# maciejkula/spotlight

Hardware: AMD Instinct MI355X
Metric: training interactions/sec, BPR dim=64 (higher is better)
Workload: dtype f32

## Files before the change

### spotlight_amd/csrc/slk_api.hip

```cpp
#include <stdarg.h>

#include <stdlib.h>

#include "slk_common.h"

static char g_create_err[512] = {0};

int slk_fail(slk_ctx *ctx, int code, const char *fmt, ...) {
    char *dst = ctx ? ctx->err : g_create_err;
    va_list ap;
    va_start(ap, fmt);
    vsnprintf(dst, 512, fmt, ap);
    va_end(ap);
    return code;
}

int slk_ensure(slk_ctx *ctx, slk_buf &b, size_t bytes) {
    if (bytes <= b.cap) return SLK_OK;
    if (b.p) {
        SLK_HIP(ctx, hipFree(b.p));
        b.p = nullptr;
        b.cap = 0;
    }
    size_t want = bytes + bytes / 8 + 256;
// ... 185 lines not shown
    SLK_OPT("sort_big_min", opt_sort_big_min, 1, SLK_OPT_MAX),
    SLK_OPT("sort_debug", opt_sort_debug, 0, 3),
    SLK_OPT("item_grid_mult", opt_item_grid_mult, 1, 4096),
    SLK_OPT("user_grid_mult", opt_user_grid_mult, 1, 4096),
    SLK_OPT("seq_variant", opt_seq_variant, 0, 1),
    SLK_OPT("explicit_fused", opt_explicit_fused, 0, 1),
    SLK_OPT("epoch_kernel", opt_epoch_kernel, 0, 1),
    SLK_OPT("item_lat_max_tiles", opt_item_lat_max_tiles, 0, SLK_OPT_MAX),
    SLK_OPT("epoch_adaptive", opt_epoch_adaptive, 0, 1),
    SLK_OPT("epoch_adaptive_max_batch", opt_epoch_adaptive_max_batch, 1, (int64_t)1 << 20),
    SLK_OPT("epoch_max_batch", opt_epoch_max_batch, 1, (int64_t)1 << 20),
    SLK_OPT("epoch_max_grid", opt_epoch_max_grid, 1, 16384),
    SLK_OPT("epoch_barrier", opt_epoch_barrier, -1, 1),
    SLK_OPT("epoch_cooperative", opt_epoch_cooperative, 0, 1),
    SLK_OPT("epoch_debug", opt_epoch_debug, 0, 63),
    SLK_OPT("epoch_dense_elems", opt_epoch_dense_elems, 0, SLK_OPT_MAX),
    SLK_OPT("user_lat_max_batch", opt_user_lat_max_batch, 0, SLK_OPT_MAX),
    SLK_OPT("item_long_gate", opt_item_long_gate, 0, 1),
    SLK_OPT("adaptive_late_min_batch", opt_adaptive_late_min_batch, 0, SLK_OPT_MAX),
    SLK_OPT("shuffle_band", opt_shuffle_band, 0, 1024),
    SLK_OPT("nt", opt_nt, 0, 63),
    SLK_OPT("record_nt_min_bytes", opt_record_nt_min_bytes, 0, SLK_OPT_MAX),
    SLK_OPT("user_bias_zero_hint", opt_user_bias_zero_hint, 0, 1),
    SLK_OPT("user_grid_own_occ", opt_user_grid_own_occ, 0, 1),
    SLK_OPT("item_single_min_items", opt_item_single_min_items, 0, SLK_OPT_MAX),
};
#undef SLK_OPT
const slk_opt_desc slk_eval_options[] = {
    {"topk_items_per_wg", 0, (int64_t)1 << 40, [](const slk_ctx *c) -> int64_t { return c->opt_topk_items_per_wg; },
     [](slk_ctx *c, int64_t v) { c->opt_topk_items_per_wg = v; }},
    {"eval_items_per_wg", 0, (int64_t)1 << 40, [](const slk_ctx *c) -> int64_t { return c->opt_eval_items_per_wg; },
     [](slk_ctx *c, int64_t v) { c->opt_eval_items_per_wg = v; }},
};
const slk_opt_desc *slk_find_option(const char *name) {
    for (const slk_opt_desc &d : slk_options)
        if (!strcmp(name, d.name)) return &d;
    for (const slk_opt_desc &d : slk_eval_options)
        if (!strcmp(name, d.name)) return &d;
    return nullptr;
}
}

SLK_EXPORT int slk_ctx_set_option(slk_ctx *ctx, const char *name, int64_t value) {
    if (!ctx || !name) return SLK_EINVAL;
    const slk_opt_desc *d = slk_find_option(name);
    if (!d || value < d->lo || value > d->hi)
        return slk_fail(ctx, SLK_EINVAL, "slk_ctx_set_option: unknown option or bad value: %s = %lld", name,
                        (long long)value);
    d->set(ctx, value);
    return SLK_OK;
}

SLK_EXPORT int slk_ctx_get_option(slk_ctx *ctx, const char *name, int64_t *value) {
    if (!ctx || !name || !value) return SLK_EINVAL;
    const slk_opt_desc *d = slk_find_option(name);
    if (!d) return slk_fail(ctx, SLK_EINVAL, "slk_ctx_get_option: unknown option %s", name);
    *value = d->get(ctx);
    return SLK_OK;
}

SLK_EXPORT int slk_ctx_get_stat(slk_ctx *ctx, const char *name, int64_t *value) {
    if (!ctx || !name || !value) return SLK_EINVAL;
    if (!strcmp(name, "shuffle_sweeps")) *value = ctx->fy_sweeps;
    else if (!strcmp(name, "shuffle_fallbacks")) *value = ctx->fy_fallbacks;
    else if (!strcmp(name, "epoch_refused")) *value = ctx->epoch_refused ? 1 : 0;
    else if (!strcmp(name, "user_long_launches")) *value = ctx->stat_user_long;
    else if (!strcmp(name, "item_long_launches")) *value = ctx->stat_item_long;
    else if (!strcmp(name, "overlapped_chunks")) *value = ctx->stat_overlapped;
    else if (!strcmp(name, "prefetched_chunks")) *value = ctx->stat_prefetched;
    else if (!strcmp(name, "shadowed_calls")) *value = ctx->stat_shadowed;
    else if (!strcmp(name, "pingpong_calls")) *value = ctx->stat_pingpong;
    else if (!strcmp(name, "single_minibatches")) *value = ctx->stat_single;
    else if (!strcmp(name, "lds_per_block")) *value = (int64_t)ctx->lds_per_block;
    else if (!strcmp(name, "lds_per_cu")) *value = (int64_t)ctx->lds_per_cu;
    else if (!strcmp(name, "prefetch_pending")) *value = !ctx->pf.valid ? 0 : (ctx->pf.all ? 2 : 1);
    else return slk_fail(ctx, SLK_EINVAL, "slk_ctx_get_stat: unknown statistic %s", name);
    return SLK_OK;
}

SLK_EXPORT int slk_profile_enable(slk_ctx *ctx, int32_t on) {
    if (!ctx) return SLK_EINVAL;
    if (!on) slk_prof_drain(ctx);
    ctx->prof_on = on != 0;
    return SLK_OK;
}

SLK_EXPORT int slk_profile_read(slk_ctx *ctx, int32_t cls, int64_t *launches, double *total_ms) {
    if (!ctx || cls < 0 || cls >= SLK_K_COUNT) return SLK_EINVAL;
    int rc = slk_prof_drain(ctx);
    if (rc) return rc;
    if (launches) *launches = ctx->prof_launches[cls];
    if (total_ms) *total_ms = ctx->prof_ms[cls];
    return SLK_OK;
}

SLK_EXPORT int slk_profile_reset(slk_ctx *ctx) {
    if (!ctx) return SLK_EINVAL;
    int rc = slk_prof_drain(ctx);
    for (int i = 0; i < SLK_K_COUNT; ++i) {
        ctx->prof_launches[i] = 0;
        ctx->prof_ms[i] = 0.0;
    }
    return rc;
}
// ... 1 lines not shown
```

### spotlight_amd/csrc/slk_bilinear.hip

```cpp
#include <math.h>

#include "slk_kernels.h"

#ifndef SLK_PP_PIPE
#define SLK_PP_PIPE 2
#endif
template <int VEC, int G, int UPD, int UMODE, bool BLOOM, bool LAT = false, bool ULONG = false, bool PP = false, bool SGL = false>
__global__ __launch_bounds__(256) void k_user_pass(slk_pass_args a) {
    static_assert(!LAT || (UMODE == 0 && !BLOOM), "LAT is the pair mode over plain tables");
    static_assert(!PP || (UMODE == 0 && !BLOOM), "PP is the pair mode over plain tables");
    static_assert(!SGL || (PP && !LAT && !ULONG && UPD == SLK_UPD_ADAGRAD), "SGL: the plain ping-pong form, Adagrad");
    static_assert(!ULONG || !BLOOM, "long user runs: plain tables");
    constexpr uint32_t S = SLK_USER_TILE;
    constexpr bool PRE = UMODE != 0;
    constexpr bool EXPL = UMODE == 2;
    __shared__ double red[256];
    constexpr int GPB = 256 / G;
    const int lane = threadIdx.x % G;
    const int grp = threadIdx.x / G;
    const int D = a.D;
    const int d0 = lane * VEC;
    const bool on = d0 < D;
    const uint32_t stride = gridDim.x * GPB;
    float loss_acc = 0.0f;
// ... 1149 lines not shown

        if (nn == 0) return SLK_OK;
        if (d_neg_in) {
            slk_prof_begin(ctx, SLK_K_SAMPLE, s);
            hipLaunchKernelGGL(k_i64_to_u32, dim3(slk_grid_for(ctx, (size_t)nc * nn, 256)), dim3(256), 0, s,
                               d_neg_in + c0 * nn, neg32, (size_t)nc * nn);
            SLK_LAUNCH_CHECK(ctx, "k_i64_to_u32");
            if (d_neg_out)
                SLK_HIP(ctx, hipMemcpyAsync(d_neg_out + c0 * nn, d_neg_in + c0 * nn, (size_t)nc * nn * 8,
                                            hipMemcpyDeviceToDevice, s));
            slk_prof_end(ctx, s);
        } else {
            if ((rc = slk_sample_u32(ctx, tables->num_items, (int64_t)nc * nn, neg32,
                                     d_neg_out ? d_neg_out + c0 * nn : nullptr, s)))
                return rc;
        }
        return SLK_OK;
    };
    auto do_sort = [&](size_t ck, slk_prep_bufs &pb, hipStream_t s) -> int {
        int rc;
        const int64_t c0 = cb[ck];
        const uint32_t nc = (uint32_t)(cb[ck + 1] - c0);
        const uint32_t nocc = nc * (uint32_t)NP;
        const int64_t *cu = d_users + c0, *ci = d_items + c0;
        const uint32_t *neg32 = neg_all ? neg_all + (size_t)c0 * nn : (const uint32_t *)pb.neg32.p;

        slk_prof_begin(ctx, SLK_K_PREP, s);
        const unsigned mbbits = slk_bits_for((uint64_t)((nc - 1) / (uint32_t)bsz));
        uint32_t *ukey_in = (uint32_t *)pb.ukey[0].p, *ukey = (uint32_t *)pb.ukey[1].p;
        const uint32_t *uit, *uk = nullptr;
        uint32_t *const ukeys[2] = {ukey_in, ukey};
        if (!pre) {
            uint64_t *const uvals[2] = {(uint64_t *)pb.uval[0].p, (uint64_t *)pb.uval[1].p};
            if ((rc = slk_sort_user_fat(ctx, cu, ci, (const uint32_t *)neg32, nc, (size_t)bsz, ubits, mbbits, ukeys, uvals, s))) return rc;
            uit = (const uint32_t *)pb.uval[1].p;
        } else {
            uint32_t *const uvals[2] = {(uint32_t *)pb.uval[0].p, (uint32_t *)pb.uval[1].p};
            if ((rc = slk_sort_user_idx(ctx, cu, nc, (size_t)bsz, ubits, mbbits, ukeys, uvals, s))) return rc;
            uk = (const uint32_t *)pb.uval[1].p;
            hipLaunchKernelGGL(k_pack_items, dim3(slk_grid_for(ctx, nc, 256)), dim3(256), 0, s, uk, ci,
                               (const uint32_t *)neg32, nc, nn, (uint32_t *)pb.uit.p);
            SLK_LAUNCH_CHECK(ctx, "k_pack_items");
            uit = (const uint32_t *)pb.uit.p;
        }
        if (late) {
            hipLaunchKernelGGL(k_invert_perm, dim3(slk_grid_for(ctx, nc, 256)), dim3(256), 0, s, uk, nc,
                               (uint32_t *)pb.ipay[0].p);
            SLK_LAUNCH_CHECK(ctx, "k_invert_perm");
        } else {
            uint32_t *const ikeys[2] = {(uint32_t *)pb.ikey[0].p, (uint32_t *)pb.ikey[1].p};
            uint32_t *const ivals[2] = {(uint32_t *)pb.ipay[0].p, (uint32_t *)pb.ipay[1].p};
            if ((rc = slk_sort_item_occ(ctx, uit, nocc, (size_t)bsz, NP, ibits, mbbits, ikeys, ivals, s))) return rc;
            if (sgl_on) {
                SLK_HIP(ctx, hipMemsetAsync(pb.mflag.p, 0, (size_t)nocc, s));
                hipLaunchKernelGGL(k_item_multi_flags, dim3(slk_grid_for(ctx, nocc, 256)), dim3(256), 0, s, (const uint32_t *)pb.ikey[1].p,
                                   (const uint32_t *)pb.ipay[1].p, nocc, (uint32_t)bsz * (uint32_t)NP, (uint8_t *)pb.msorted.p,
                                   (uint8_t *)pb.mflag.p);
                SLK_LAUNCH_CHECK(ctx, "k_item_multi_flags");
            }
        }
        if (!epoch_route) {
            const uint32_t n_mb_c = (nc + (uint32_t)bsz - 1) / (uint32_t)bsz;
            if ((rc = slk_ensure(ctx, pb.lflags, 2 * (size_t)n_mb_c * 4))) return rc;
            SLK_HIP(ctx, hipMemsetAsync(pb.lflags.p, 0, 2 * (size_t)n_mb_c * 4, s));
            if (!late) {
                hipLaunchKernelGGL(k_item_long_flags, dim3(slk_grid_for(ctx, nocc / (4 * gpb) + n_mb_c, 256)), dim3(256), 0, s,
                                   (const uint32_t *)pb.ikey[1].p, nocc, (uint32_t)bsz * (uint32_t)NP, 4u * gpb,
// ... 494 lines not shown
```

### spotlight_amd/csrc/slk_common.h

```cpp
#pragma once
#include <hip/hip_runtime.h>
#include <stdint.h>
#include <stdio.h>
#include <string.h>

#include <vector>

#include "../../include/spotlight_hip.h"

#define SLK_EAGAIN_EPOCH 1
#define SLK_EXPORT extern "C" __attribute__((visibility("default")))

#if defined(__HIPCC__)
#define SLK_WAVES_PER_EU(n) __attribute__((amdgpu_waves_per_eu(n, n)))
#define SLK_WAVES_PER_EU_RANGE(lo, hi) __attribute__((amdgpu_waves_per_eu(lo, hi)))
#else
#define SLK_WAVES_PER_EU(n)
#define SLK_WAVES_PER_EU_RANGE(lo, hi)
#endif

#if defined(__HIPCC__)
#define SLK_DRAIN_VMEM() asm volatile("s_waitcnt vmcnt(0)" ::: "memory")
#else
#define SLK_DRAIN_VMEM() ((void)0)
// ... 55 lines not shown
    hipEvent_t a, b;
};

struct slk_ctx {
    int device = 0;
    int num_cus = 256;
    size_t lds_per_block = (size_t)160 * 1024;
    size_t lds_per_cu = (size_t)160 * 1024;
    char err[512] = {0};
    hipStream_t last_stream = nullptr;
    slk_rng_dev *d_rng = nullptr;
    uint32_t *d_jump[2] = {nullptr, nullptr};
    bool mt_attr_set = false;
    slk_buf bias_shadow;
    float *shadow_src_p = nullptr, *shadow_src_s = nullptr;
    int64_t shadow_rows = 0;
    bool shadow_active = false;
    slk_buf pp_alt, pp_flags;
    float *pp_src_u = nullptr;
    int64_t pp_rows = 0;
    int pp_dim = 0;
    bool pp_active = false;
    slk_buf mt_tmp;

    slk_buf raw, cnt, neg32, ukey[2], uval[2], uit, ikey[2], ipay[2], gk, sk, snap, losspart,
        sort_tmp, dgrad[4], ipart, ipart_meta, upart_meta;
    size_t dgrad_elems[4] = {0, 0, 0, 0};
    int64_t opt_chunk_interactions = (int64_t)1 << 23;
    int opt_overlap_prep = 0;
    int64_t opt_mt_long_min_blocks = 16385;
    int opt_prefetch_wait = 0;
    int64_t opt_overlap_min_batch = (int64_t)1 << 16;
    int64_t opt_sort_big_min = (int64_t)1 << 20;
    int opt_sort_debug = 0;
    int opt_item_grid_mult = 128;
    int opt_user_grid_mult = 8;
    int opt_seq_variant = 1;
    int64_t opt_adaptive_late_min_batch = (int64_t)1 << 18;
    int64_t opt_user_lat_max_batch = (int64_t)1 << 17;
    int64_t opt_item_lat_max_tiles = 2048;
    int opt_item_long_gate = 1;
    int opt_explicit_fused = 1;
    int opt_epoch_kernel = 1;
    int64_t opt_epoch_max_batch = 1024;
    bool epoch_refused = false;
    int opt_epoch_adaptive = 1;
    int64_t opt_epoch_adaptive_max_batch = 1024;
    int epoch_bars_per_mb = 2;
    int opt_epoch_barrier = -1;
    int opt_epoch_cooperative = 0;
    int opt_epoch_debug = 0;
    int opt_epoch_max_grid = 256;
    int64_t opt_epoch_dense_elems = (int64_t)1 << 18;
    void *h_coef[2] = {nullptr, nullptr};
    size_t h_coef_cap[2] = {0, 0};
    hipEvent_t ev_coef[2] = {nullptr, nullptr};
    int coef_flip = 0;
    int opt_nt = 3;
    int64_t opt_item_single_min_items = (int64_t)1 << 24;
    int opt_user_grid_own_occ = 0;
    int64_t opt_topk_items_per_wg = 0;
    int64_t opt_eval_items_per_wg = 0;
    int opt_user_bias_zero_hint = 1;
    int64_t opt_record_nt_min_bytes = (int64_t)192 << 20;
    slk_prep_bufs pb[2];
    hipStream_t prep_stream = nullptr;
// ... 7 lines not shown
    int64_t sh_n = 0;
    int sh_M = 0, sh_S = 0, sh_world = 0;
    int sh_NP = 2;
    bool sh_adaptive = false;
    unsigned sh_ubits = 0;
    std::vector<int64_t> sh_ustart, sh_rstart;
    std::vector<int64_t> sh_sslots, sh_rslots;
    std::vector<uint64_t> sh_host, sh_host2;

    int64_t ts_rows = -1, ts_nseg = 0;
    int ts_L = 0, ts_step = 0;

    int64_t em_occ = -1, em_rows = 0, em_segments = -1;
    int em_dim = 0;

    struct {
        bool valid = false;
        int set = 0;
        const void *users = nullptr, *items = nullptr;
        int64_t n = 0, bsz = 0, nc0 = 0;
        int loss = 0, nn = 0;
        bool all = false;
    } pf;
    slk_buf pf_neg;
    slk_buf call_neg;
    int64_t stat_overlapped = 0;
    int64_t stat_prefetched = 0;
    int64_t stat_shadowed = 0;
    int64_t stat_pingpong = 0;
    int64_t stat_single = 0;
    int last_pipe_set = -1;
    uint32_t ipart_gen = 0;
    uint32_t upart_gen = 0;
    int64_t stat_user_long = 0, stat_item_long = 0;
    int fy_sweeps = 0;
    int fy_fallbacks = 0;
    int opt_shuffle_band = 1;

    bool prof_on = false;
    std::vector<slk_prof_span> spans;
    std::vector<hipEvent_t> ev_pool;
    std::vector<std::pair<const void *, int>> occ_cache;
    int64_t prof_launches[SLK_K_COUNT] = {0};
    double prof_ms[SLK_K_COUNT] = {0};
};

int slk_fail(slk_ctx *ctx, int code, const char *fmt, ...);
int slk_ensure(slk_ctx *ctx, slk_buf &b, size_t bytes);
int slk_ensure_lflags_host(slk_ctx *ctx, slk_prep_bufs &pb, size_t n);
void slk_prof_begin(slk_ctx *ctx, int cls, hipStream_t s);
void slk_prof_end(slk_ctx *ctx, hipStream_t s);
int slk_prof_drain(slk_ctx *ctx);
int slk_prep_stream_init(slk_ctx *ctx);
hipStream_t slk_copy_stream(slk_ctx *ctx);

#define SLK_HIP(ctx, call)                                                                   \
    do {                                                                                     \
        hipError_t e_ = (call);                                                              \
        if (e_ != hipSuccess)                                                                \
            return slk_fail((ctx), SLK_EIO, "%s failed: %s (%s:%d)", #call, hipGetErrorString(e_), \
                            __FILE__, __LINE__);                                             \
    } while (0)

#define SLK_LAUNCH_CHECK(ctx, what)                                                          \
    do {                                                                                     \
        hipError_t e_ = hipGetLastError();                                                   \
        if (e_ != hipSuccess)                                                                \
            return slk_fail((ctx), SLK_EIO, "launch of %s failed: %s", (what), hipGetErrorString(e_)); \
    } while (0)

#define SLK_MT_JUMP_BLOCKS 64
#define SLK_MT_JUMP_LEVELS 2
static inline int slk_mt_jump_blocks(int level) { return level ? 4 * SLK_MT_JUMP_BLOCKS : SLK_MT_JUMP_BLOCKS; }
#define SLK_MT_JUMP_WG 256
static_assert(SLK_MT_JUMP_WG * SLK_MT_JUMP_BLOCKS + 1 == 16385, "slk_ctx::opt_mt_long_min_blocks");
#define SLK_MT_JUMP_TERMS 10752
#define SLK_MT_JUMP_PAD (33 * 624 - 1)
const uint32_t *slk_mt_jump_table(slk_ctx *ctx, int level);

int slk_sample_u32(slk_ctx *ctx, int64_t num_items, int64_t count, uint32_t *d_out32, int64_t *d_out64,
                   hipStream_t s);

int slk_sort_pairs_u32_u32(slk_ctx *ctx, const uint32_t *kin, uint32_t *kout, const uint32_t *vin,
                           uint32_t *vout, size_t n, unsigned end_bit, hipStream_t s, bool clobber = false);
int slk_sort_pairs_u32_u32_in(slk_ctx *ctx, slk_buf &scratch, const uint32_t *kin, uint32_t *kout, const uint32_t *vin,
                              uint32_t *vout, size_t n, unsigned end_bit, hipStream_t s, bool clobber = false);
int slk_sort_pairs_u64_u32_in(slk_ctx *ctx, slk_buf &scratch, const uint64_t *kin, uint64_t *kout, const uint32_t *vin,
                              uint32_t *vout, size_t n, unsigned end_bit, hipStream_t s, bool clobber = false);
int slk_sort_pairs_u32_u64(slk_ctx *ctx, const uint32_t *kin, uint32_t *kout, const uint64_t *vin,
                           uint64_t *vout, size_t n, unsigned end_bit, hipStream_t s, bool clobber = false);
int slk_sort_fy_steps(slk_ctx *ctx, slk_buf &scratch, const uint32_t *J, uint32_t n, uint32_t *const key[2], uint32_t *const val[2],
                      hipStream_t s);
int slk_sort_pairs_any(slk_ctx *ctx, int kind, const void *kin, void *kout, const void *vin, void *vout, size_t n, size_t seg_len,
                       unsigned bits, hipStream_t s, bool clobber);
int slk_sort_user_fat(slk_ctx *ctx, const int64_t *users, const int64_t *items, const uint32_t *neg32, size_t nc, size_t bsz,
                      unsigned ubits, unsigned mbbits, uint32_t *const key[2], uint64_t *const val[2], hipStream_t s);
int slk_sort_user_idx(slk_ctx *ctx, const int64_t *users, size_t nc, size_t bsz, unsigned ubits, unsigned mbbits,
                      uint32_t *const key[2], uint32_t *const val[2], hipStream_t s);
int slk_sort_item_occ(slk_ctx *ctx, const uint32_t *uit, size_t nocc, size_t bsz, int NP, unsigned ibits, unsigned mbbits,
                      uint32_t *const key[2], uint32_t *const val[2], hipStream_t s);

int slk_eval_predict_all(slk_ctx *ctx, const slk_tables *tables, const float *rep, const float *rbias, const int64_t *gmap,
                         float *d_out, hipStream_t s);
int slk_eval_user_rep(slk_ctx *ctx, const slk_tables *tables, int vec, int g, const int64_t *d_user, const float **rep,
                      const float **rbias, const int64_t **gmap, hipStream_t s);

int slk_check_tables(slk_ctx *ctx, const slk_tables *t, unsigned table_mask, int *vec, int *g, bool shadow_ok = false,
                     bool pingpong_ok = false);
int slk_launch_i64_to_u32(slk_ctx *ctx, const int64_t *in, uint32_t *out, size_t n, hipStream_t s);

int slk_sort_reserve(slk_ctx *ctx, size_t n);
int slk_compact_heads(slk_ctx *ctx, const uint32_t *d_sorted, uint32_t n, uint32_t *d_heads, uint32_t *d_segid,
                      uint32_t *nseg_out, hipStream_t s);
bool slk_epoch_eligible(const slk_ctx *ctx, const slk_tables *tables, const slk_optim *optim, int64_t bsz, int loss, bool bloom);
int slk_epoch_reserve(slk_ctx *ctx, const slk_tables *tables, const slk_optim *optim, uint32_t n_mb, int64_t bsz, int loss, int NP);
int slk_epoch_run_chunk(slk_ctx *ctx, const slk_tables *tables, slk_optim *optim, const slk_prep_bufs &pb, uint32_t nc,
                        int64_t bsz, unsigned ubits, unsigned ibits, int loss, int NP, int RS, float *snap, float *gsn,
                        float *d_mb_loss, const float *d_ratings, hipStream_t s);
int slk_mt_generate_blocks(slk_ctx *ctx, unsigned long long nblocks, hipStream_t s);
int slk_sample_reserve(slk_ctx *ctx, int64_t num_items, int64_t count);
int slk_mt_jump_reserve(slk_ctx *ctx, int level);
int slk_mt_level_for(const slk_ctx *ctx, unsigned long long nblocks);
int slk_rng_write_state(slk_ctx *ctx, const uint32_t *h_key, int32_t pos);

static inline unsigned slk_bits_for(uint64_t max_value) {
    unsigned b = 1;
    while (b < 64 && (max_value >> b)) ++b;
    return b;
}
// ... 181 lines not shown
```

### spotlight_amd/csrc/slk_sort.hip

```cpp
#include "slk_common.h"

namespace {

constexpr int RS_RB = 8;
constexpr int RS_RADIX = 1 << RS_RB;
constexpr uint32_t RS_VAL_MASK = (1u << 30) - 1u;
constexpr uint32_t RS_AGG = 1u, RS_INC = 2u;
constexpr int RS_MAX_PASS = 8;
constexpr int RS_HIST_KEYS = 8192;
constexpr int RS_LBW = 16;
constexpr uint32_t RS_MAX_SPINS = 1u << 22;

enum { RS_LOAD_PLAIN = 0, RS_LOAD_USER_FAT, RS_LOAD_USER_IDX, RS_LOAD_ITEM_OCC, RS_LOAD_FY_STEPS };

struct rs_args {
    const void *kin, *vin;
    void *kout, *vout;
    const int64_t *users, *items;
    const uint32_t *neg32, *uit;
    uint32_t n, seg_len, tps, ntiles, hbps;
    uint32_t kseg;
    unsigned idbits;
    uint32_t fy_n;
    int npass, pass;
    int shift[RS_MAX_PASS], width[RS_MAX_PASS];
    uint32_t *hist, *base;
    uint32_t *ticket;
    uint32_t *status;
    int32_t *abort_flag;
    int xcd;
    uint32_t nseg;
    int debug;
};

template <class KeyT>
__device__ __forceinline__ uint32_t rs_digit(KeyT k, int shift, uint32_t mask) {
    return (uint32_t)(k >> shift) & mask;
}

template <class KeyT, class ValT, int LOADER>
__device__ __forceinline__ void rs_load(const rs_args &a, uint32_t gi, uint32_t seg, KeyT &k, ValT &v) {
    if (LOADER == RS_LOAD_FY_STEPS) {
        const uint32_t i = a.fy_n - 1u - gi, j = a.uit[gi];
        k = (KeyT)(j == i ? a.fy_n : j);
        v = (ValT)i;
        return;
    }
    if (LOADER != RS_LOAD_PLAIN && a.kseg) seg = gi / a.kseg;
    if (LOADER == RS_LOAD_PLAIN) {
        k = ((const KeyT *)a.kin)[gi];
        v = ((const ValT *)a.vin)[gi];
    } else if (LOADER == RS_LOAD_USER_FAT) {
        k = (KeyT)((seg << a.idbits) | (uint32_t)a.users[gi]);
        v = (ValT)(((uint64_t)a.neg32[gi] << 32) | (uint64_t)(uint32_t)a.items[gi]);
    } else if (LOADER == RS_LOAD_USER_IDX) {
        k = (KeyT)((seg << a.idbits) | (uint32_t)a.users[gi]);
        v = (ValT)gi;
    } else {
        k = (KeyT)((seg << a.idbits) | a.uit[gi]);
        v = (ValT)gi;
    }
}

template <class KeyT, int LOADER>
__device__ __forceinline__ KeyT rs_load_key(const rs_args &a, uint32_t gi, uint32_t seg) {
    if (LOADER == RS_LOAD_PLAIN) return ((const KeyT *)a.kin)[gi];
    if (LOADER == RS_LOAD_FY_STEPS) {
        const uint32_t j = a.uit[gi];
        return (KeyT)(j == a.fy_n - 1u - gi ? a.fy_n : j);
    }
    if (a.kseg) seg = gi / a.kseg;
    if (LOADER == RS_LOAD_ITEM_OCC) return (KeyT)((seg << a.idbits) | a.uit[gi]);
    return (KeyT)((seg << a.idbits) | (uint32_t)a.users[gi]);
}

template <class KeyT, int LOADER>
__global__ __launch_bounds__(256) void k_rs_hist(rs_args a) {
    __shared__ uint32_t sh[RS_MAX_PASS * RS_RADIX];
    const uint32_t seg = blockIdx.x / a.hbps, hb = blockIdx.x - seg * a.hbps;
    const uint32_t s0 = seg * a.seg_len;
    const uint32_t s1 = (a.n - s0 < a.seg_len) ? a.n : s0 + a.seg_len;
    const uint32_t b0 = s0 + hb * (uint32_t)RS_HIST_KEYS;
    const uint32_t b1 = (b0 >= s1 || s1 - b0 < (uint32_t)RS_HIST_KEYS) ? s1 : b0 + (uint32_t)RS_HIST_KEYS;
    for (int i = threadIdx.x; i < a.npass * RS_RADIX; i += 256) sh[i] = 0u;
    __syncthreads();
    for (uint32_t g0 = b0 + threadIdx.x; g0 < b1; g0 += 8u * 256u) {
        KeyT k[8];
#pragma unroll
        for (int u = 0; u < 8; ++u) {
            const uint32_t gi = g0 + (uint32_t)u * 256u;
            k[u] = gi < b1 ? rs_load_key<KeyT, LOADER>(a, gi, seg) : (KeyT)0;
        }
#pragma unroll
        for (int u = 0; u < 8; ++u) {
            if (g0 + (uint32_t)u * 256u >= b1) continue;
            for (int p = 0; p < a.npass; ++p)
                atomicAdd(&sh[p * RS_RADIX + rs_digit<KeyT>(k[u], a.shift[p], (1u << a.width[p]) - 1u)], 1u);
        }
// ... 52 lines not shown

__device__ __forceinline__ bool rs_walk(const rs_args &a, const uint32_t *row0, uint32_t radix, uint32_t tis, uint32_t &before) {
    int32_t t = (int32_t)tis - 1;
    uint32_t spins = 0;
    bool done = false;
    while (!done) {
        uint32_t v[RS_LBW];
#pragma unroll
        for (int i = 0; i < RS_LBW; ++i) {
            const int32_t ti = t - i;
            v[i] = ti >= 0 ? __hip_atomic_load(row0 + (size_t)ti * radix, __ATOMIC_RELAXED, __HIP_MEMORY_SCOPE_AGENT) : 0u;
        }
        int consumed = 0;
#pragma unroll
        for (int i = 0; i < RS_LBW; ++i) {
            const uint32_t f = v[i] >> 30;
            if (done || f == 0u || consumed != i) continue;
            before += v[i] & RS_VAL_MASK;
            ++consumed;
            if (f == RS_INC) done = true;
        }
        t -= consumed;
        if (!done && consumed == 0) {
            if (++spins > RS_MAX_SPINS) {
                *a.abort_flag = 1;
                return false;
            }
            __builtin_amdgcn_s_sleep(1);
        }
    }
    return true;
}

template <class KeyT, class ValT, int THREADS, int KPT, int LOADER, bool SINGLE>
__global__ __launch_bounds__(THREADS) SLK_WAVES_PER_EU_RANGE(4, 6) void k_rs_scatter(rs_args a) {
    constexpr int WAVES = THREADS / 64, KW = WAVES, TILE = KW * 64 * KPT;
    constexpr int OPT = (TILE + THREADS - 1) / THREADS;
    constexpr int XB = sizeof(KeyT) > sizeof(ValT) ? sizeof(KeyT) : sizeof(ValT);
    __shared__ uint32_t s_cnt[KW * RS_RADIX];
    __shared__ uint32_t s_lbase[RS_RADIX];
    __shared__ uint32_t s_goff[RS_RADIX];
    __shared__ uint32_t s_wsum[WAVES];
    __shared__ uint32_t s_tile;
    __shared__ __attribute__((aligned(16))) unsigned char s_x[(size_t)TILE * XB];

    const int lane = threadIdx.x & 63, wave = threadIdx.x >> 6;
    constexpr bool is_key = true;
    const int shift = a.shift[a.pass], nbits = a.width[a.pass];
    const uint32_t radix = 1u << nbits, dmask = radix - 1u;
    if (!SINGLE && threadIdx.x == 0) {
        if (a.xcd) {
            const uint32_t x0 = rs_xcc_id();
            uint32_t t = 0xffffffffu;
            for (uint32_t i = 0; i < 8u && t == 0xffffffffu; ++i) {
                const uint32_t x = (x0 + i) & 7u;
                const uint32_t nsx = a.nseg > x ? (a.nseg - x + 7u) / 8u : 0u;
                if (!nsx) continue;
                const uint32_t k = atomicAdd(a.ticket + 8 + a.pass * 8 + x, 1u);
                if (k < nsx * a.tps) t = (x + 8u * (k / a.tps)) * a.tps + k % a.tps;
            }
            s_tile = t;
        } else {
            s_tile = atomicAdd(a.ticket + a.pass, 1u);
        }
    }
    for (int i = threadIdx.x; i < KW * RS_RADIX; i += THREADS) s_cnt[i] = 0u;
    if (threadIdx.x < RS_RADIX) s_lbase[threadIdx.x] = 0u;
    __syncthreads();
    const uint32_t tile = SINGLE ? 0u : s_tile;
    if (tile == 0xffffffffu) return;
    const uint32_t seg = tile / a.tps, tis = tile - seg * a.tps;
    const uint32_t s0 = seg * a.seg_len;
    const uint32_t s1 = (a.n - s0 < a.seg_len) ? a.n : s0 + a.seg_len;
    const uint32_t t0 = s0 + tis * (uint32_t)TILE;
    const uint32_t cnt = t0 >= s1 ? 0u : ((s1 - t0 < (uint32_t)TILE) ? s1 - t0 : (uint32_t)TILE);

    KeyT key[KPT];
    ValT val[KPT];
    uint32_t pos2[KPT / 2];
    const uint32_t e0 = (uint32_t)wave * 64u * KPT + (uint32_t)lane;
    if (is_key) {
        if (LOADER == RS_LOAD_PLAIN) {
#pragma unroll
            for (int j = 0; j < KPT; ++j) {
                const uint32_t e = e0 + (uint32_t)j * 64u;
                key[j] = e < cnt ? ((const KeyT *)a.kin)[t0 + e] : (KeyT)0;
            }
#pragma unroll
            for (int j = 0; j < KPT; ++j) {
                const uint32_t e = e0 + (uint32_t)j * 64u;
                val[j] = e < cnt ? ((const ValT *)a.vin)[t0 + e] : (ValT)0;
            }
        } else {
#pragma unroll
            for (int j = 0; j < KPT; ++j) {
                const uint32_t e = e0 + (uint32_t)j * 64u;
                key[j] = 0;
                val[j] = 0;
                if (e < cnt) rs_load<KeyT, ValT, LOADER>(a, t0 + e, seg, key[j], val[j]);
            }
        }
        if (!SINGLE) {
#pragma unroll
            for (int j = 0; j < KPT; ++j)
                if (e0 + (uint32_t)j * 64u < cnt) atomicAdd(&s_lbase[rs_digit<KeyT>(key[j], shift, dmask)], 1u);
        }
    } else {
#pragma unroll
        for (int j = 0; j < KPT; ++j) {
            key[j] = 0;
            val[j] = 0;
        }
    }
    if (!SINGLE) __syncthreads();

    uint32_t tcount = 0, before = 0;
    uint32_t *wcnt = s_cnt + (is_key ? wave : 0) * RS_RADIX;
    auto rank_keys = [&]() {
#pragma unroll
        for (int j = 0; j < KPT; ++j) {
            if ((j & 1) == 0) pos2[j / 2] = 0u;
            if ((uint32_t)wave * 64u * KPT + (uint32_t)j * 64u >= cnt) continue;
            const bool valid = e0 + (uint32_t)j * 64u < cnt;
            const uint32_t dj = rs_digit<KeyT>(key[j], shift, dmask);
            uint32_t r;
            if (a.debug & 2) {
                r = valid ? atomicAdd(&wcnt[dj], 1u) : 0u;
            } else {
                const unsigned long long m = rs_match(dj, nbits, valid);
                const int leader = m ? __ffsll((long long)m) - 1 : lane;
                uint32_t first = 0;
                if (m && lane == leader) first = atomicAdd(&wcnt[dj], (uint32_t)__popcll(m));
                first = __shfl(first, leader);
                r = first + (uint32_t)__popcll(m & ((1ull << lane) - 1ull));
            }
            pos2[j / 2] = (j & 1) ? (pos2[j / 2] | (r << 16)) : r;
        }
    };
    {
        const uint32_t d = threadIdx.x;
        if (!SINGLE && d < radix) {
            tcount = s_lbase[d];
            __hip_atomic_store(a.status + (size_t)tile * radix + d, ((tis == 0 ? RS_INC : RS_AGG) << 30) | tcount, __ATOMIC_RELAXED,
                               __HIP_MEMORY_SCOPE_AGENT);
// ... 14 lines not shown
            }
            if (SINGLE) tcount = run;
        }
        const uint32_t lb = rs_block_excl_scan<THREADS>(tcount, s_wsum);
        if (d < radix) {
            uint32_t gbase = lb;
            if (!SINGLE) gbase = a.base[((size_t)seg * a.npass + a.pass) * RS_RADIX + d];
            s_lbase[d] = lb;
            s_goff[d] = gbase + before - lb;
        }
    }
    __syncthreads();
    KeyT *xk = reinterpret_cast<KeyT *>(s_x);
    if (is_key) {
#pragma unroll
        for (int j = 0; j < KPT; ++j) {
            if (e0 + (uint32_t)j * 64u < cnt) {
                const uint32_t dj = rs_digit<KeyT>(key[j], shift, dmask);
                const uint32_t pj = ((pos2[j / 2] >> ((j & 1) * 16)) & 0xffffu) + s_lbase[dj] + wcnt[dj];
                pos2[j / 2] = (j & 1) ? ((pos2[j / 2] & 0xffffu) | (pj << 16)) : ((pos2[j / 2] & 0xffff0000u) | pj);
                xk[pj] = key[j];
            }
        }
    }
    __syncthreads();
    uint32_t gidx[OPT];
#pragma unroll
    for (int j = 0; j < OPT; ++j) {
        const uint32_t i = (uint32_t)j * THREADS + threadIdx.x;
        gidx[j] = 0;
        if (i < cnt) {
            const KeyT k = xk[i];
            gidx[j] = s_goff[rs_digit<KeyT>(k, shift, dmask)] + i;
            ((KeyT *)a.kout)[gidx[j]] = k;
        }
    }
    __syncthreads();
    ValT *xv = reinterpret_cast<ValT *>(s_x);
    if (is_key) {
#pragma unroll
        for (int j = 0; j < KPT; ++j)
            if (e0 + (uint32_t)j * 64u < cnt) xv[(pos2[j / 2] >> ((j & 1) * 16)) & 0xffffu] = val[j];
    }
    __syncthreads();
#pragma unroll
    for (int j = 0; j < OPT; ++j) {
        const uint32_t i = (uint32_t)j * THREADS + threadIdx.x;
        if (i < cnt) ((ValT *)a.vout)[gidx[j]] = xv[i];
    }
}

struct rs_plan {
    uint32_t n = 0, seg_len = 0, nseg = 0, tps = 0, ntiles = 0, hbps = 0;
    int npass = 0, shift[RS_MAX_PASS], width[RS_MAX_PASS];
    size_t off_ticket = 0, off_status[RS_MAX_PASS], zero_bytes = 0, off_base = 0, off_data = 0, ctl_bytes = 0;
};

static void rs_split_bits(unsigned bits, int *npass, int *shift, int *width) {
    int P = (int)((bits + RS_RB - 1) / RS_RB);
    if (P < 1) P = 1;
    const int lo = (int)bits / P, rem = (int)bits % P;
    int s = 0;
    for (int p = 0; p < P; ++p) {
        width[p] = lo + (p < rem ? 1 : 0);
        if (width[p] < 1) width[p] = 1;
        shift[p] = s;
        s += width[p];
    }
    *npass = P;
}

static void rs_make_plan(rs_plan &pl, size_t n, size_t seg_len, unsigned bits, unsigned tile) {
    pl.n = (uint32_t)n;
    pl.seg_len = (uint32_t)(seg_len && seg_len < n ? seg_len : n);
    pl.nseg = (uint32_t)((n + pl.seg_len - 1) / pl.seg_len);
    pl.tps = (pl.seg_len + tile - 1) / tile;
    pl.ntiles = pl.nseg * pl.tps;
    pl.hbps = (pl.seg_len + RS_HIST_KEYS - 1) / RS_HIST_KEYS;
    rs_split_bits(bits, &pl.npass, pl.shift, pl.width);
    size_t o = (size_t)pl.nseg * pl.npass * RS_RADIX * 4;
    pl.off_ticket = o;
    o += 512;
    for (int p = 0; p < pl.npass; ++p) {
        pl.off_status[p] = o;
        o += (size_t)pl.ntiles * ((size_t)1 << pl.width[p]) * 4;
    }
    pl.zero_bytes = o;
    o = (o + 255) & ~(size_t)255;
    pl.off_base = o;
    o += (size_t)pl.nseg * pl.npass * RS_RADIX * 4;
    pl.off_data = (o + 255) & ~(size_t)255;
    pl.ctl_bytes = pl.off_data;
}

#ifndef RS_BIG_THREADS
#define RS_BIG_THREADS 512
#endif
#ifndef RS_BIG_KPT
#define RS_BIG_KPT 16
#endif

template <class KeyT, class ValT, int LOADER>
struct rs_kernels {
    static void launch(int cfg, bool single, unsigned grid, hipStream_t s, const rs_args &a) {
        if (single)
            hipLaunchKernelGGL((k_rs_scatter<KeyT, ValT, 256, 16, RS_LOAD_PLAIN, true>), dim3(1), dim3(256), 0, s, a);
        else if (cfg == 1)
            hipLaunchKernelGGL((k_rs_scatter<KeyT, ValT, RS_BIG_THREADS, RS_BIG_KPT, LOADER, false>), dim3(grid), dim3(RS_BIG_THREADS), 0, s, a);
        else
            hipLaunchKernelGGL((k_rs_scatter<KeyT, ValT, 256, 16, LOADER, false>), dim3(grid), dim3(256), 0, s, a);
    }
};

static inline unsigned rs_tile_of(int cfg) { return cfg == 1 ? (unsigned)(RS_BIG_THREADS * RS_BIG_KPT) : 4096u; }

template <class KeyT, class ValT, int LOADER>
static int rs_sort(slk_ctx *ctx, slk_buf &scratch, rs_args a, size_t n, size_t seg_len, unsigned bits, void *kalt, void *valt,
                   hipStream_t s) {
    if (n == 0) return SLK_OK;
    if (n >= ((size_t)1 << 31)) return slk_fail(ctx, SLK_EINVAL, "sort of %zu pairs: at most 2^31 - 1", n);
    if (bits > 8 * sizeof(KeyT)) bits = 8 * sizeof(KeyT);
    if (bits < 1) bits = 1;
    const bool single = LOADER == RS_LOAD_PLAIN && n <= 4096 && (seg_len == 0 || seg_len >= n);
    const int cfg = (!single && n >= (size_t)ctx->opt_sort_big_min) ? 1 : 0;
    const unsigned tile = rs_tile_of(cfg);
    rs_plan pl;
    rs_make_plan(pl, n, single ? 0 : seg_len, bits, tile);
    if (pl.seg_len >= (1u << 30)) return slk_fail(ctx, SLK_EINVAL, "sort segment of %u pairs: at most 2^30 - 1", pl.seg_len);
    const bool inplace0 = kalt && kalt == a.kin && (pl.npass & 1) == 0;
    const bool need_tmp = pl.npass > 1 && (!kalt || inplace0);
    const size_t koff = pl.off_data, voff = (koff + n * sizeof(KeyT) + 255) & ~(size_t)255;
    int rc = slk_ensure(ctx, scratch, need_tmp ? voff + n * sizeof(ValT) : pl.ctl_bytes);
    if (rc) return rc;
    char *base = (char *)scratch.p;
    void *k0dst = nullptr, *v0dst = nullptr;
    if (need_tmp && !kalt) {
        kalt = base + koff;
        valt = base + voff;
    } else if (inplace0) {
        k0dst = base + koff;
        v0dst = base + voff;
    }
    a.n = pl.n;
    a.seg_len = pl.seg_len;
    a.tps = pl.tps;
    a.ntiles = pl.ntiles;
    a.hbps = pl.hbps;
    a.npass = pl.npass;
    for (int p = 0; p < pl.npass; ++p) {
        a.shift[p] = pl.shift[p];
        a.width[p] = pl.width[p];
    }
    a.hist = (uint32_t *)base;
    a.base = (uint32_t *)(base + pl.off_base);
    a.ticket = (uint32_t *)(base + pl.off_ticket);
    a.abort_flag = &ctx->d_rng->sort_abort;
    a.debug = ctx->opt_sort_debug;
    a.nseg = pl.nseg;
    a.xcd = pl.nseg >= 2 ? 1 : 0;
    void *kfinal = a.kout, *vfinal = a.vout;
    if (!single) {
        SLK_HIP(ctx, hipMemsetAsync(base, 0, pl.zero_bytes, s));
        a.pass = 0;
        hipLaunchKernelGGL((k_rs_hist<KeyT, LOADER>), dim3(pl.nseg * pl.hbps), dim3(256), 0, s, a);
        SLK_LAUNCH_CHECK(ctx, "k_rs_hist");
        hipLaunchKernelGGL(k_rs_scan, dim3(pl.nseg * (unsigned)pl.npass), dim3(256), 0, s, a);
        SLK_LAUNCH_CHECK(ctx, "k_rs_scan");
    }
    for (int p = 0; p < pl.npass; ++p) {
        const bool to_final = ((pl.npass - 1 - p) & 1) == 0;
        a.pass = p;
        a.kout = to_final ? kfinal : kalt;
        a.vout = to_final ? vfinal : valt;
        if (p == 0 && k0dst) {
            a.kout = k0dst;
            a.vout = v0dst;
        }
        a.status = (uint32_t *)(base + pl.off_status[p]);
        if (p == 0)
            rs_kernels<KeyT, ValT, LOADER>::launch(cfg, single, pl.ntiles, s, a);
        else
            rs_kernels<KeyT, ValT, RS_LOAD_PLAIN>::launch(cfg, single, pl.ntiles, s, a);
        SLK_LAUNCH_CHECK(ctx, "k_rs_scatter");
        a.kin = a.kout;
        a.vin = a.vout;
    }
    return SLK_OK;
}

}

int slk_sort_pairs_u32_u32_in(slk_ctx *ctx, slk_buf &scratch, const uint32_t *kin, uint32_t *kout, const uint32_t *vin,
                              uint32_t *vout, size_t n, unsigned end_bit, hipStream_t s, bool clobber) {
    rs_args a;
    memset(&a, 0, sizeof(a));
    a.kin = kin;
    a.vin = vin;
    a.kout = kout;
    a.vout = vout;
    return rs_sort<uint32_t, uint32_t, RS_LOAD_PLAIN>(ctx, scratch, a, n, 0, end_bit, clobber ? (void *)kin : nullptr,
                                                      clobber ? (void *)vin : nullptr, s);
}

int slk_sort_pairs_u64_u32_in(slk_ctx *ctx, slk_buf &scratch, const uint64_t *kin, uint64_t *kout, const uint32_t *vin,
                              uint32_t *vout, size_t n, unsigned end_bit, hipStream_t s, bool clobber) {
    rs_args a;
    memset(&a, 0, sizeof(a));
    a.kin = kin;
    a.vin = vin;
    a.kout = kout;
    a.vout = vout;
    return rs_sort<uint64_t, uint32_t, RS_LOAD_PLAIN>(ctx, scratch, a, n, 0, end_bit, clobber ? (void *)kin : nullptr,
                                                      clobber ? (void *)vin : nullptr, s);
}

// ... 25 lines not shown
    return rs_sort<uint32_t, uint32_t, RS_LOAD_FY_STEPS>(ctx, scratch, a, (size_t)n - 1, 0, slk_bits_for((uint64_t)n), key[0], val[0], s);
}

int slk_sort_pairs_any(slk_ctx *ctx, int kind, const void *kin, void *kout, const void *vin, void *vout, size_t n, size_t seg_len,
                       unsigned bits, hipStream_t s, bool clobber) {
    rs_args a;
    memset(&a, 0, sizeof(a));
    a.kin = kin;
    a.vin = vin;
    a.kout = kout;
    a.vout = vout;
    void *ka = clobber ? (void *)kin : nullptr, *va = clobber ? (void *)vin : nullptr;
    if (kind == 0) return rs_sort<uint32_t, uint32_t, RS_LOAD_PLAIN>(ctx, ctx->sort_tmp, a, n, seg_len, bits, ka, va, s);
    if (kind == 1) return rs_sort<uint32_t, uint64_t, RS_LOAD_PLAIN>(ctx, ctx->sort_tmp, a, n, seg_len, bits, ka, va, s);
    if (kind == 2) return rs_sort<uint64_t, uint32_t, RS_LOAD_PLAIN>(ctx, ctx->sort_tmp, a, n, seg_len, bits, ka, va, s);
    return slk_fail(ctx, SLK_EINVAL, "slk_sort_pairs_any: kind %d", kind);
}

static bool rs_segmented(size_t n, size_t seg_len) { return seg_len < n && seg_len >= 32768; }

template <class KeyT, class ValT, int LOADER>
static int rs_sort_fused(slk_ctx *ctx, rs_args a, size_t n, size_t seg_len, unsigned idbits, unsigned mbbits, void *const key[2],
                         void *const val[2], hipStream_t s) {
    a.idbits = idbits;
    a.kout = key[1];
    a.vout = val[1];
    const bool seg = rs_segmented(n, seg_len), one = seg_len >= n;
    a.kseg = seg ? 0u : (uint32_t)seg_len;
    return rs_sort<KeyT, ValT, LOADER>(ctx, ctx->sort_tmp, a, n, seg ? seg_len : 0, (seg || one) ? idbits : idbits + mbbits, key[0],
                                       val[0], s);
}

int slk_sort_user_fat(slk_ctx *ctx, const int64_t *users, const int64_t *items, const uint32_t *neg32, size_t nc, size_t bsz,
                      unsigned ubits, unsigned mbbits, uint32_t *const key[2], uint64_t *const val[2], hipStream_t s) {
    rs_args a;
    memset(&a, 0, sizeof(a));
    a.users = users;
    a.items = items;
    a.neg32 = neg32;
    return rs_sort_fused<uint32_t, uint64_t, RS_LOAD_USER_FAT>(ctx, a, nc, bsz, ubits, mbbits, (void *const *)key, (void *const *)val, s);
}

int slk_sort_user_idx(slk_ctx *ctx, const int64_t *users, size_t nc, size_t bsz, unsigned ubits, unsigned mbbits,
                      uint32_t *const key[2], uint32_t *const val[2], hipStream_t s) {
    rs_args a;
    memset(&a, 0, sizeof(a));
    a.users = users;
    return rs_sort_fused<uint32_t, uint32_t, RS_LOAD_USER_IDX>(ctx, a, nc, bsz, ubits, mbbits, (void *const *)key, (void *const *)val, s);
}

int slk_sort_item_occ(slk_ctx *ctx, const uint32_t *uit, size_t nocc, size_t bsz, int NP, unsigned ibits, unsigned mbbits,
                      uint32_t *const key[2], uint32_t *const val[2], hipStream_t s) {
    rs_args a;
    memset(&a, 0, sizeof(a));
    a.uit = uit;
    return rs_sort_fused<uint32_t, uint32_t, RS_LOAD_ITEM_OCC>(ctx, a, nocc, bsz * (size_t)NP, ibits, mbbits, (void *const *)key,
                                                               (void *const *)val, s);
}

int slk_sort_reserve(slk_ctx *ctx, size_t n) {
    if (n == 0) return SLK_OK;
    rs_plan pl;
    rs_make_plan(pl, n, 0, 32, 4096);
    size_t need = pl.ctl_bytes;
    need += (size_t)pl.ntiles * RS_RADIX * 4 * 4;
    return slk_ensure(ctx, ctx->sort_tmp, need);
}
```

Baseline: 1.579 billion.

## Pack user, item and negative into one 64-bit sort key for user sort

```diff
diff --git a/spotlight_amd/csrc/slk_api.hip b/spotlight_amd/csrc/slk_api.hip
--- a/spotlight_amd/csrc/slk_api.hip
+++ b/spotlight_amd/csrc/slk_api.hip
@@ -241,8 +241,14 @@
     {"eval_items_per_wg", 0, (int64_t)1 << 40, [](const slk_ctx *c) -> int64_t { return c->opt_eval_items_per_wg; },
      [](slk_ctx *c, int64_t v) { c->opt_eval_items_per_wg = v; }},
 };
+const slk_opt_desc slk_sort_options[] = {
+    {"sort_user_packed", 0, 1, [](const slk_ctx *c) -> int64_t { return c->opt_sort_user_packed; },
+     [](slk_ctx *c, int64_t v) { c->opt_sort_user_packed = (int)v; }},
+};
 const slk_opt_desc *slk_find_option(const char *name) {
     for (const slk_opt_desc &d : slk_options)
+        if (!strcmp(name, d.name)) return &d;
+    for (const slk_opt_desc &d : slk_sort_options)
         if (!strcmp(name, d.name)) return &d;
     for (const slk_opt_desc &d : slk_eval_options)
         if (!strcmp(name, d.name)) return &d;
@@ -279,6 +285,7 @@
     else if (!strcmp(name, "prefetched_chunks")) *value = ctx->stat_prefetched;
     else if (!strcmp(name, "shadowed_calls")) *value = ctx->stat_shadowed;
     else if (!strcmp(name, "pingpong_calls")) *value = ctx->stat_pingpong;
+    else if (!strcmp(name, "sort_user_packed_sorts")) *value = ctx->stat_sort_user_packed;
     else if (!strcmp(name, "single_minibatches")) *value = ctx->stat_single;
     else if (!strcmp(name, "lds_per_block")) *value = (int64_t)ctx->lds_per_block;
     else if (!strcmp(name, "lds_per_cu")) *value = (int64_t)ctx->lds_per_cu;
diff --git a/spotlight_amd/csrc/slk_bilinear.hip b/spotlight_amd/csrc/slk_bilinear.hip
--- a/spotlight_amd/csrc/slk_bilinear.hip
+++ b/spotlight_amd/csrc/slk_bilinear.hip
@@ -1205,7 +1205,7 @@
         uint32_t *const ukeys[2] = {ukey_in, ukey};
         if (!pre) {
             uint64_t *const uvals[2] = {(uint64_t *)pb.uval[0].p, (uint64_t *)pb.uval[1].p};
-            if ((rc = slk_sort_user_fat(ctx, cu, ci, (const uint32_t *)neg32, nc, (size_t)bsz, ubits, mbbits, ukeys, uvals, s))) return rc;
+            if ((rc = slk_sort_user_fat(ctx, cu, ci, (const uint32_t *)neg32, nc, (size_t)bsz, ubits, bloom ? 0u : ibits, mbbits, ukeys, uvals, s))) return rc;
             uit = (const uint32_t *)pb.uval[1].p;
         } else {
             uint32_t *const uvals[2] = {(uint32_t *)pb.uval[0].p, (uint32_t *)pb.uval[1].p};
diff --git a/spotlight_amd/csrc/slk_common.h b/spotlight_amd/csrc/slk_common.h
--- a/spotlight_amd/csrc/slk_common.h
+++ b/spotlight_amd/csrc/slk_common.h
@@ -111,6 +111,7 @@
     int opt_prefetch_wait = 0;
     int64_t opt_overlap_min_batch = (int64_t)1 << 16;
     int64_t opt_sort_big_min = (int64_t)1 << 20;
+    int opt_sort_user_packed = 1;
     int opt_sort_debug = 0;
     int opt_item_grid_mult = 128;
     int opt_user_grid_mult = 8;
@@ -184,6 +185,7 @@
     int last_pipe_set = -1;
     uint32_t ipart_gen = 0;
     uint32_t upart_gen = 0;
+    int64_t stat_sort_user_packed = 0;
     int64_t stat_user_long = 0, stat_item_long = 0;
     int fy_sweeps = 0;
     int fy_fallbacks = 0;
@@ -246,7 +248,7 @@
 int slk_sort_pairs_any(slk_ctx *ctx, int kind, const void *kin, void *kout, const void *vin, void *vout, size_t n, size_t seg_len,
                        unsigned bits, hipStream_t s, bool clobber);
 int slk_sort_user_fat(slk_ctx *ctx, const int64_t *users, const int64_t *items, const uint32_t *neg32, size_t nc, size_t bsz,
-                      unsigned ubits, unsigned mbbits, uint32_t *const key[2], uint64_t *const val[2], hipStream_t s);
+                      unsigned ubits, unsigned ibits, unsigned mbbits, uint32_t *const key[2], uint64_t *const val[2], hipStream_t s);
 int slk_sort_user_idx(slk_ctx *ctx, const int64_t *users, size_t nc, size_t bsz, unsigned ubits, unsigned mbbits,
                       uint32_t *const key[2], uint32_t *const val[2], hipStream_t s);
 int slk_sort_item_occ(slk_ctx *ctx, const uint32_t *uit, size_t nocc, size_t bsz, int NP, unsigned ibits, unsigned mbbits,
diff --git a/spotlight_amd/csrc/slk_sort.hip b/spotlight_amd/csrc/slk_sort.hip
--- a/spotlight_amd/csrc/slk_sort.hip
+++ b/spotlight_amd/csrc/slk_sort.hip
@@ -1,4 +1,6 @@
 #include "slk_common.h"
+
+#include <type_traits>
 
 namespace {
 
@@ -11,7 +13,9 @@
 constexpr int RS_LBW = 16;
 constexpr uint32_t RS_MAX_SPINS = 1u << 22;
 
-enum { RS_LOAD_PLAIN = 0, RS_LOAD_USER_FAT, RS_LOAD_USER_IDX, RS_LOAD_ITEM_OCC, RS_LOAD_FY_STEPS };
+enum { RS_LOAD_PLAIN = 0, RS_LOAD_USER_FAT, RS_LOAD_USER_IDX, RS_LOAD_ITEM_OCC, RS_LOAD_FY_STEPS, RS_LOAD_USER_PACK };
+
+struct rs_none {};
 
 struct rs_args {
     const void *kin, *vin;
@@ -21,6 +25,7 @@
     uint32_t n, seg_len, tps, ntiles, hbps;
     uint32_t kseg;
     unsigned idbits;
+    unsigned pbits;
     uint32_t fy_n;
     int npass, pass;
     int shift[RS_MAX_PASS], width[RS_MAX_PASS];
@@ -40,30 +45,33 @@
 
 template <class KeyT, class ValT, int LOADER>
 __device__ __forceinline__ void rs_load(const rs_args &a, uint32_t gi, uint32_t seg, KeyT &k, ValT &v) {
-    if (LOADER == RS_LOAD_FY_STEPS) {
+    if constexpr (LOADER == RS_LOAD_USER_PACK) {
+        k = ((KeyT)(uint32_t)a.users[gi] << (2u * a.pbits)) | ((KeyT)(uint32_t)a.items[gi] << a.pbits) | (KeyT)a.neg32[gi];
+    } else if constexpr (LOADER == RS_LOAD_FY_STEPS) {
         const uint32_t i = a.fy_n - 1u - gi, j = a.uit[gi];
         k = (KeyT)(j == i ? a.fy_n : j);
         v = (ValT)i;
-        return;
-    }
-    if (LOADER != RS_LOAD_PLAIN && a.kseg) seg = gi / a.kseg;
-    if (LOADER == RS_LOAD_PLAIN) {
+    } else if constexpr (LOADER == RS_LOAD_PLAIN) {
         k = ((const KeyT *)a.kin)[gi];
         v = ((const ValT *)a.vin)[gi];
-    } else if (LOADER == RS_LOAD_USER_FAT) {
-        k = (KeyT)((seg << a.idbits) | (uint32_t)a.users[gi]);
-        v = (ValT)(((uint64_t)a.neg32[gi] << 32) | (uint64_t)(uint32_t)a.items[gi]);
-    } else if (LOADER == RS_LOAD_USER_IDX) {
-        k = (KeyT)((seg << a.idbits) | (uint32_t)a.users[gi]);
-        v = (ValT)gi;
     } else {
-        k = (KeyT)((seg << a.idbits) | a.uit[gi]);
-        v = (ValT)gi;
+        if (a.kseg) seg = gi / a.kseg;
+        if (LOADER == RS_LOAD_USER_FAT) {
+            k = (KeyT)((seg << a.idbits) | (uint32_t)a.users[gi]);
+            v = (ValT)(((uint64_t)a.neg32[gi] << 32) | (uint64_t)(uint32_t)a.items[gi]);
+        } else if (LOADER == RS_LOAD_USER_IDX) {
+            k = (KeyT)((seg << a.idbits) | (uint32_t)a.users[gi]);
+            v = (ValT)gi;
+        } else {
+            k = (KeyT)((seg << a.idbits) | a.uit[gi]);
+            v = (ValT)gi;
+        }
     }
 }
 
 template <class KeyT, int LOADER>
 __device__ __forceinline__ KeyT rs_load_key(const rs_args &a, uint32_t gi, uint32_t seg) {
+    if constexpr (LOADER == RS_LOAD_USER_PACK) return (KeyT)(uint32_t)a.users[gi] << (2u * a.pbits);
     if (LOADER == RS_LOAD_PLAIN) return ((const KeyT *)a.kin)[gi];
     if (LOADER == RS_LOAD_FY_STEPS) {
         const uint32_t j = a.uit[gi];
@@ -182,10 +190,11 @@
     return true;
 }
 
-template <class KeyT, class ValT, int THREADS, int KPT, int LOADER, bool SINGLE>
+template <class KeyT, class ValT, int THREADS, int KPT, int LOADER, bool SINGLE, bool UNPACK = false>
 __global__ __launch_bounds__(THREADS) SLK_WAVES_PER_EU_RANGE(4, 6) void k_rs_scatter(rs_args a) {
     constexpr int WAVES = THREADS / 64, KW = WAVES, TILE = KW * 64 * KPT;
     constexpr int OPT = (TILE + THREADS - 1) / THREADS;
+    constexpr bool HASV = !std::is_same<ValT, rs_none>::value;
     constexpr int XB = sizeof(KeyT) > sizeof(ValT) ? sizeof(KeyT) : sizeof(ValT);
     __shared__ uint32_t s_cnt[KW * RS_RADIX];
     __shared__ uint32_t s_lbase[RS_RADIX];
@@ -230,23 +239,25 @@
     uint32_t pos2[KPT / 2];
     const uint32_t e0 = (uint32_t)wave * 64u * KPT + (uint32_t)lane;
     if (is_key) {
-        if (LOADER == RS_LOAD_PLAIN) {
+        if constexpr (LOADER == RS_LOAD_PLAIN) {
 #pragma unroll
             for (int j = 0; j < KPT; ++j) {
                 const uint32_t e = e0 + (uint32_t)j * 64u;
                 key[j] = e < cnt ? ((const KeyT *)a.kin)[t0 + e] : (KeyT)0;
             }
-#pragma unroll
-            for (int j = 0; j < KPT; ++j) {
-                const uint32_t e = e0 + (uint32_t)j * 64u;
-                val[j] = e < cnt ? ((const ValT *)a.vin)[t0 + e] : (ValT)0;
+            if constexpr (HASV) {
+#pragma unroll
+                for (int j = 0; j < KPT; ++j) {
+                    const uint32_t e = e0 + (uint32_t)j * 64u;
+                    val[j] = e < cnt ? ((const ValT *)a.vin)[t0 + e] : (ValT)0;
+                }
             }
         } else {
 #pragma unroll
             for (int j = 0; j < KPT; ++j) {
                 const uint32_t e = e0 + (uint32_t)j * 64u;
                 key[j] = 0;
-                val[j] = 0;
+                val[j] = ValT();
                 if (e < cnt) rs_load<KeyT, ValT, LOADER>(a, t0 + e, seg, key[j], val[j]);
             }
         }
@@ -259,7 +270,7 @@
 #pragma unroll
         for (int j = 0; j < KPT; ++j) {
             key[j] = 0;
-            val[j] = 0;
+            val[j] = ValT();
         }
     }
     if (!SINGLE) __syncthreads();
@@ -340,21 +351,29 @@
         if (i < cnt) {
             const KeyT k = xk[i];
             gidx[j] = s_goff[rs_digit<KeyT>(k, shift, dmask)] + i;
-            ((KeyT *)a.kout)[gidx[j]] = k;
-        }
-    }
-    __syncthreads();
-    ValT *xv = reinterpret_cast<ValT *>(s_x);
-    if (is_key) {
-#pragma unroll
-        for (int j = 0; j < KPT; ++j)
-            if (e0 + (uint32_t)j * 64u < cnt) xv[(pos2[j / 2] >> ((j & 1) * 16)) & 0xffffu] = val[j];
-    }
-    __syncthreads();
-#pragma unroll
-    for (int j = 0; j < OPT; ++j) {
-        const uint32_t i = (uint32_t)j * THREADS + threadIdx.x;
-        if (i < cnt) ((ValT *)a.vout)[gidx[j]] = xv[i];
+            if constexpr (UNPACK) {
+                const uint32_t im = (1u << a.pbits) - 1u;
+                ((uint32_t *)a.kout)[gidx[j]] = (seg << a.idbits) | (uint32_t)(k >> (2u * a.pbits));
+                ((uint64_t *)a.vout)[gidx[j]] = ((uint64_t)((uint32_t)k & im) << 32) | (uint64_t)((uint32_t)(k >> a.pbits) & im);
+            } else {
+                ((KeyT *)a.kout)[gidx[j]] = k;
+            }
+        }
+    }
+    if constexpr (HASV) {
+        __syncthreads();
+        ValT *xv = reinterpret_cast<ValT *>(s_x);
+        if (is_key) {
+#pragma unroll
+            for (int j = 0; j < KPT; ++j)
+                if (e0 + (uint32_t)j * 64u < cnt) xv[(pos2[j / 2] >> ((j & 1) * 16)) & 0xffffu] = val[j];
+        }
+        __syncthreads();
+#pragma unroll
+        for (int j = 0; j < OPT; ++j) {
+            const uint32_t i = (uint32_t)j * THREADS + threadIdx.x;
+            if (i < cnt) ((ValT *)a.vout)[gidx[j]] = xv[i];
+        }
     }
 }
 
@@ -364,11 +383,11 @@
     size_t off_ticket = 0, off_status[RS_MAX_PASS], zero_bytes = 0, off_base = 0, off_data = 0, ctl_bytes = 0;
 };
 
-static void rs_split_bits(unsigned bits, int *npass, int *shift, int *width) {
+static void rs_split_bits(unsigned bits, unsigned base, int *npass, int *shift, int *width) {
     int P = (int)((bits + RS_RB - 1) / RS_RB);
     if (P < 1) P = 1;
     const int lo = (int)bits / P, rem = (int)bits % P;
-    int s = 0;
+    int s = (int)base;
     for (int p = 0; p < P; ++p) {
         width[p] = lo + (p < rem ? 1 : 0);
         if (width[p] < 1) width[p] = 1;
@@ -378,14 +397,14 @@
     *npass = P;
 }
 
-static void rs_make_plan(rs_plan &pl, size_t n, size_t seg_len, unsigned bits, unsigned tile) {
+static void rs_make_plan(rs_plan &pl, size_t n, size_t seg_len, unsigned bits, unsigned tile, unsigned base = 0) {
     pl.n = (uint32_t)n;
     pl.seg_len = (uint32_t)(seg_len && seg_len < n ? seg_len : n);
     pl.nseg = (uint32_t)((n + pl.seg_len - 1) / pl.seg_len);
     pl.tps = (pl.seg_len + tile - 1) / tile;
     pl.ntiles = pl.nseg * pl.tps;
     pl.hbps = (pl.seg_len + RS_HIST_KEYS - 1) / RS_HIST_KEYS;
-    rs_split_bits(bits, &pl.npass, pl.shift, pl.width);
+    rs_split_bits(bits, base, &pl.npass, pl.shift, pl.width);
     size_t o = (size_t)pl.nseg * pl.npass * RS_RADIX * 4;
     pl.off_ticket = o;
     o += 512;
@@ -410,8 +429,17 @@
 
 template <class KeyT, class ValT, int LOADER>
 struct rs_kernels {
-    static void launch(int cfg, bool single, unsigned grid, hipStream_t s, const rs_args &a) {
-        if (single)
+    static void launch(int cfg, bool single, bool unpack, unsigned grid, hipStream_t s, const rs_args &a) {
+        if constexpr (std::is_same<ValT, rs_none>::value) {
+            if (unpack && cfg == 1)
+                hipLaunchKernelGGL((k_rs_scatter<KeyT, ValT, RS_BIG_THREADS, RS_BIG_KPT, LOADER, false, true>), dim3(grid), dim3(RS_BIG_THREADS), 0, s, a);
+            else if (unpack)
+                hipLaunchKernelGGL((k_rs_scatter<KeyT, ValT, 256, 16, LOADER, false, true>), dim3(grid), dim3(256), 0, s, a);
+            else if (cfg == 1)
+                hipLaunchKernelGGL((k_rs_scatter<KeyT, ValT, RS_BIG_THREADS, RS_BIG_KPT, LOADER, false>), dim3(grid), dim3(RS_BIG_THREADS), 0, s, a);
+            else
+                hipLaunchKernelGGL((k_rs_scatter<KeyT, ValT, 256, 16, LOADER, false>), dim3(grid), dim3(256), 0, s, a);
+        } else if (single)
             hipLaunchKernelGGL((k_rs_scatter<KeyT, ValT, 256, 16, RS_LOAD_PLAIN, true>), dim3(1), dim3(256), 0, s, a);
         else if (cfg == 1)
             hipLaunchKernelGGL((k_rs_scatter<KeyT, ValT, RS_BIG_THREADS, RS_BIG_KPT, LOADER, false>), dim3(grid), dim3(RS_BIG_THREADS), 0, s, a);
@@ -424,16 +452,17 @@
 
 template <class KeyT, class ValT, int LOADER>
 static int rs_sort(slk_ctx *ctx, slk_buf &scratch, rs_args a, size_t n, size_t seg_len, unsigned bits, void *kalt, void *valt,
-                   hipStream_t s) {
+                   hipStream_t s, unsigned kbase = 0) {
+    constexpr bool PACKED = LOADER == RS_LOAD_USER_PACK;
     if (n == 0) return SLK_OK;
     if (n >= ((size_t)1 << 31)) return slk_fail(ctx, SLK_EINVAL, "sort of %zu pairs: at most 2^31 - 1", n);
-    if (bits > 8 * sizeof(KeyT)) bits = 8 * sizeof(KeyT);
+    if (bits + kbase > 8 * sizeof(KeyT)) bits = 8 * sizeof(KeyT) - kbase;
     if (bits < 1) bits = 1;
     const bool single = LOADER == RS_LOAD_PLAIN && n <= 4096 && (seg_len == 0 || seg_len >= n);
     const int cfg = (!single && n >= (size_t)ctx->opt_sort_big_min) ? 1 : 0;
     const unsigned tile = rs_tile_of(cfg);
     rs_plan pl;
-    rs_make_plan(pl, n, single ? 0 : seg_len, bits, tile);
+    rs_make_plan(pl, n, single ? 0 : seg_len, bits, tile, kbase);
     if (pl.seg_len >= (1u << 30)) return slk_fail(ctx, SLK_EINVAL, "sort segment of %u pairs: at most 2^30 - 1", pl.seg_len);
     const bool inplace0 = kalt && kalt == a.kin && (pl.npass & 1) == 0;
     const bool need_tmp = pl.npass > 1 && (!kalt || inplace0);
@@ -484,11 +513,13 @@
             a.kout = k0dst;
             a.vout = v0dst;
         }
+        const bool unpack = PACKED && p == pl.npass - 1;
+        if (PACKED && !unpack) a.kout = to_final ? vfinal : kalt;
         a.status = (uint32_t *)(base + pl.off_status[p]);
         if (p == 0)
-            rs_kernels<KeyT, ValT, LOADER>::launch(cfg, single, pl.ntiles, s, a);
+            rs_kernels<KeyT, ValT, LOADER>::launch(cfg, single, unpack, pl.ntiles, s, a);
         else
-            rs_kernels<KeyT, ValT, RS_LOAD_PLAIN>::launch(cfg, single, pl.ntiles, s, a);
+            rs_kernels<KeyT, ValT, RS_LOAD_PLAIN>::launch(cfg, single, unpack, pl.ntiles, s, a);
         SLK_LAUNCH_CHECK(ctx, "k_rs_scatter");
         a.kin = a.kout;
         a.vin = a.vout;
@@ -580,12 +611,21 @@
 }
 
 int slk_sort_user_fat(slk_ctx *ctx, const int64_t *users, const int64_t *items, const uint32_t *neg32, size_t nc, size_t bsz,
-                      unsigned ubits, unsigned mbbits, uint32_t *const key[2], uint64_t *const val[2], hipStream_t s) {
+                      unsigned ubits, unsigned ibits, unsigned mbbits, uint32_t *const key[2], uint64_t *const val[2], hipStream_t s) {
     rs_args a;
     memset(&a, 0, sizeof(a));
     a.users = users;
     a.items = items;
     a.neg32 = neg32;
+    const bool seg = rs_segmented(nc, bsz);
+    if (ctx->opt_sort_user_packed && ibits && (seg || bsz >= nc) && ubits + 2 * ibits <= 64) {
+        ++ctx->stat_sort_user_packed;
+        a.idbits = ubits;
+        a.pbits = ibits;
+        a.kout = key[1];
+        a.vout = val[1];
+        return rs_sort<uint64_t, rs_none, RS_LOAD_USER_PACK>(ctx, ctx->sort_tmp, a, nc, seg ? bsz : 0, ubits, val[0], nullptr, s, 2 * ibits);
+    }
     return rs_sort_fused<uint32_t, uint64_t, RS_LOAD_USER_FAT>(ctx, a, nc, bsz, ubits, mbbits, (void *const *)key, (void *const *)val, s);
 }
 
```

Measured after the change: 1.593 billion (median of 6 runs). No clear change (+0.9%).
